# privefl/bigsnpr

Measured on AMD Instinct MI355X. Metric: SNP-cols/sec for bed_randomSVD k=20 (m*passes/wall), higher is better.
Workload: dtype i8 (2-bit codes x 24-bit (early block steps) / 16-bit (late block steps) fixed-point image of the fp64 basis in int8 slices, exact int32 MFMA accumulation; fp64 panel algebra and Rayleigh-Ritz)

## Files before the change

bigsnpr_amd/csrc/bsn_internal.hpp:

```cpp
#pragma once
#include <hip/hip_runtime.h>
#include <stdint.h>

#include <atomic>
#include <cstdarg>
#include <cstdio>
#include <functional>
#include <cstdlib>
#include <memory>
#include <stdexcept>
#include <string>
#include <vector>

#include "bigsnpr_hip.h"

namespace bsn {
inline const char *abl_getenv(const char *name) {
#ifdef BSN_ABLATION
  return getenv(name);
#else
  (void)name;
  return nullptr;
#endif
}
// ... 85 lines not shown
  void *comm = nullptr;
  int rank = 0, world = 1, device = 0;
  hipStream_t stream = nullptr;
  std::atomic<int> aborted{0};
  bool timing = false;
  struct Timed { hipEvent_t a, b; int cls; };
  std::vector<Timed> timed;
  std::vector<hipEvent_t> ev_pool;
  ~bsn_comm() {
    for (auto &t : timed) { (void)hipEventDestroy(t.a); (void)hipEventDestroy(t.b); }
    for (auto e : ev_pool) (void)hipEventDestroy(e);
  }
};

constexpr int kProfKinds = 6;
struct bsn_op {
  bsn_bed *bed = nullptr;
  int64_t n = 0, m = 0;
  bool rows_identity = true;
  bool cols_contig = true;
  bool no_na = false;
  bool na_skip_c = false, na_skip_p = false;
  bool stats_pending = false;
  bsn::DevBuf<int32_t> d_counts;
  bsn::DevBuf<int32_t> d_na;
  long long *h_na_total = nullptr;
  bool na_poll = false;
  int64_t col0 = 0;
  int slices = 4;
  int64_t passes = 0;
  const double *late_center = nullptr, *late_scale = nullptr;
  const double *preq_X = nullptr;
  int64_t preq_ldx = 0;
  int preq_nvec = 0, preq_S = 0;
  bool profile = false;
  int prof_kind_override = -1;
  std::vector<hipEvent_t> ev_begin, ev_end;
  std::vector<int> ev_kind;
  std::vector<char> ev_more;
  const void *prof_kernel[kProfKinds] = {};
  const void *last_kernel = nullptr;
  ~bsn_op() {
    for (auto e : ev_begin) (void)hipEventDestroy(e);
    for (auto e : ev_end) (void)hipEventDestroy(e);
    if (h_na_total) (void)hipHostFree(h_na_total);
  }
  bsn::DevBuf<int32_t> d_rows;
  bsn::DevBuf<int32_t> d_cols;
  bsn::DevBuf<double> d_center, d_scale;
  bsn::DevBuf<double> d_xfull;
  bsn::DevBuf<int8_t> d_q;
  bsn::DevBuf<int32_t> d_acc;
  bsn::DevBuf<double> d_meta;
  bsn::DevBuf<double> d_yfull;
};

struct bsn_bed {
  int64_t n = 0, m = 0, n_byte = 0, pitch = 0;
  int bits = 2;
  double v_off = 0.0, v_step = 1.0;
  bool generic = false;
  double *d_lut = nullptr;
  uint8_t *d_img = nullptr;
  uint8_t *d_tiled = nullptr;
  bool tiled_tried = false;
  size_t tiled_cap = 0;
  const uint8_t *h_map = nullptr;
  void *map_base = nullptr;
  size_t map_len = 0;
  int64_t slab_cols = 0;
  int fd_file = -1;
  bsn_bed *slab_img = nullptr;
  void *slab_stage = nullptr;
  bool streamed() const { return d_img == nullptr && h_map != nullptr; }
  uint8_t *d_smaj = nullptr;
  int64_t pitch_smaj = 0, rows_smaj = 0;
  bool smaj_tried = false;
  size_t smaj_cap = 0;
  void *smaj_job = nullptr;
  int64_t cap_m = 0;
  bsn_bed *sub = nullptr;
  uint64_t sub_key = 0;
  std::vector<int64_t> sub_cols, sub_rows;
  bool last_solve_on_sub = false;
  int device = 0;
  bool stream_borrowed = false;
  hipStream_t stream = nullptr;
  hipStream_t stream_up = nullptr;
  hipEvent_t ev_up = nullptr;
  hipEvent_t ev0 = nullptr, ev1 = nullptr;
  std::vector<int32_t> na_cnt;
  struct CountsCache {
    std::vector<int64_t> rows;
    std::vector<int32_t> cnt;
    void clear() {
      rows.clear();
      cnt.clear();
    }
  } counts_cache;
  struct StatsCache {
    bsn::DevBuf<int32_t> d_cnt;
    std::vector<uint8_t> known;
    int64_t n_known = 0;
    bsn::DevBuf<int32_t> d_cols;
    uint64_t cols_key = 0;
    void clear() {
// ... 141 lines not shown
```

bigsnpr_amd/csrc/matvec.hip:

```cpp
#include <cmath>
#include <cstdlib>

#include "bsn_internal.hpp"
#include "prodt_sparse.hpp"
#include <type_traits>

namespace bsn {

typedef int v4i __attribute__((ext_vector_type(4)));
typedef int v8i __attribute__((ext_vector_type(8)));

static thread_local const void *g_last_kernel = nullptr;
#define BSN_KLAUNCH(kern, ...)                 \
  do {                                         \
    g_last_kernel = (const void *)(kern);      \
    hipLaunchKernelGGL(kern, __VA_ARGS__);     \
  } while (0)

__device__ __forceinline__ uint32_t lut4(uint32_t lut, uint32_t sel) {
  return __builtin_amdgcn_perm(lut, lut, sel);
}
__device__ __forceinline__ uint32_t perm8(uint32_t hi, uint32_t lo, uint32_t sel) {
  return __builtin_amdgcn_perm(hi, lo, sel);
}

constexpr uint32_t kLutG0 = 0x00020100u;
constexpr uint32_t kLutNA = 0x01000000u;
constexpr uint32_t kLutHom2 = 0x00010000u;
constexpr uint32_t kLutHet = 0x00000100u;
constexpr uint32_t kLutRaw = 0xFFFFFFFFu;

struct VecMeta {
  unsigned long long absmax_bits;
  long long sum_hi, sum_lo;
  long long sum2_hi, sum2_lo;
  unsigned long long nonfinite;
  double qscale;
  double pad;
};
static_assert(sizeof(VecMeta) == 64, "VecMeta layout");

__global__ void k_meta_clear(VecMeta *meta, int nvec) {
  int v = blockIdx.x * blockDim.x + threadIdx.x;
  if (v < nvec) {
    VecMeta z = {};
    meta[v] = z;
  }
}

__global__ void k_scatter_rows(const double *X, int64_t ldx, const int32_t *rows, int64_t n,
                               double *xfull, int64_t ldf) {
  int64_t i = (int64_t)blockIdx.x * blockDim.x + threadIdx.x;
  int v = blockIdx.y;
  if (i >= n) return;
  atomicAdd(&xfull[(int64_t)rows[i] + v * ldf], X[i + v * ldx]);
}

// ... 129 lines not shown
#ifdef BSN_ABLATION
      const bool sm = (raw3 >> 8) == 2;
      const long long sgA = A < 0 ? -1 : 1, sgB = B < 0 ? -1 : 1;
      long long mA = A < 0 ? -A : A, mB = B < 0 ? -B : B;
#endif
#pragma unroll
      for (int s = 0; s < S; s++) {
#ifdef BSN_ABLATION
        const int8_t da = sm ? (int8_t)(sgA * (mA & 0x7F)) : (int8_t)(A & 0xFF), db = sm ? (int8_t)(sgB * (mB & 0x7F)) : (int8_t)(B & 0xFF);
        mA >>= 7;
        mB >>= 7;
#else
        const int8_t da = (int8_t)(A & 0xFF), db = (int8_t)(B & 0xFF);
#endif
        A = (A - da) >> 8;
        B = (B - db) >> 8;
        if constexpr (PERM == 2) {
          const int r = prodt_sparse_row(e), ba = prodt_sparse_byte(e, 0), bb = prodt_sparse_byte(e, 1);
          pk[r][s][ba >> 2] |= (uint32_t)(uint8_t)da << (8 * (ba & 3));
          pk[r][s][bb >> 2] |= (uint32_t)(uint8_t)db << (8 * (bb & 3));
        } else {
          pk[0][s][pos >> 2] |= (uint32_t)(uint8_t)da << (8 * (pos & 3));
          pk[1][s][pos >> 2] |= (uint32_t)(uint8_t)db << (8 * (pos & 3));
        }
      }
    }
    for (int p = 0; p < nplanes; p++)
#pragma unroll
      for (int s = 0; s < S; s++) {
#ifdef BSN_ABLATION
        const int col = (raw3 >> 8) == 1 ? s * (int)gridDim.y + v : v * S + s;
#else
        const int col = v * S + s;
#endif
        int8_t *dst = q + ((kb * nplanes + p) * ncol + col) * 16;
        *(uint4 *)dst = p == 0 ? uint4{pk[0][s][0], pk[0][s][1], pk[0][s][2], pk[0][s][3]}
                               : uint4{pk[1][s][0], pk[1][s][1], pk[1][s][2], pk[1][s][3]};
      }
  }
  for (int off = 32; off > 0; off >>= 1) {
    shi += __shfl_down(shi, off); slo += __shfl_down(slo, off);
    shi2 += __shfl_down(shi2, off); slo2 += __shfl_down(slo2, off);
  }
  if (tid == 0) {
    atomicAdd((unsigned long long *)&meta[v].sum_hi, (unsigned long long)shi);
    atomicAdd((unsigned long long *)&meta[v].sum_lo, (unsigned long long)slo);
    if (mode >= 1) {
      atomicAdd((unsigned long long *)&meta[v].sum2_hi, (unsigned long long)shi2);
      atomicAdd((unsigned long long *)&meta[v].sum2_lo, (unsigned long long)slo2);
    }
  }
}

template <int NB, int NPLANE, int KC, bool RAW0, bool STATS, bool CONTIG, int ABL = 0, int TILES = 2,
          int WAVES = 8, int MINW = 1, int TAG = 0, bool TILED = false, int SGB = 0, bool NASKIP = false>
__global__ __launch_bounds__(64 * WAVES, MINW) void k_cprod(const uint8_t *__restrict__ img, int64_t pitch,
                                               const int32_t *__restrict__ cols, int64_t col0,
                                               int64_t m, const int8_t *__restrict__ xq,
                                               int32_t *__restrict__ acc_out, int64_t m_out,
                                               uint32_t lutA, uint32_t lutB, uint32_t lutC,
                                               int32_t *__restrict__ counts, int32_t n_pad_samples) {
  constexpr int NCOL = 16 * NB;
  constexpr int LD = KC / 256;
  constexpr int XS = KC / 16 * NCOL;
  __shared__ uint4 xs[2][XS];
  const int tid = threadIdx.x, wave = tid >> 6, lane = tid & 63;
  const int c = lane & 15, g = lane >> 4;
  constexpr int NT = 64 * WAVES;
  const int64_t wg_base = (int64_t)blockIdx.x * (WAVES * 16 * TILES);
  const int64_t snp_base = wg_base + wave * (16 * TILES);
  const uint8_t *rowp[TILES];
  uint32_t voff[TILES];
#pragma unroll
  for (int t = 0; t < TILES; t++) {
    int64_t j = snp_base + t * 16 + c;
    if (j > m - 1) j = m - 1;
    int64_t col = CONTIG ? col0 + j : (int64_t)cols[j];
    rowp[t] = img + col * pitch + g * 16;
    voff[t] = TILED ? (uint32_t)((((j - wg_base) >> 6) * (pitch >> 8)) * 16384 + (j & 63) * 256 + g * 16)
                    : (uint32_t)((j - wg_base) * pitch + g * 16);
  }
  static_assert(!TILED || (CONTIG && (WAVES * 16 * TILES) % 64 == 0), "streaming layout: whole 64-variant blocks");
  const __amdgpu_buffer_rsrc_t rs = __builtin_amdgcn_make_buffer_rsrc(
      (void *)(TILED ? img + (((col0 + wg_base) >> 6) * (pitch >> 8)) * 16384
                     : img + (col0 + (CONTIG ? wg_base : 0)) * pitch),
      0, 0x7fffffff, 0x00020000);
  typedef unsigned int v4u __attribute__((ext_vector_type(4)));
  auto gload = [&](const int t, const int off) -> uint4 {
    if constexpr (CONTIG) {
      constexpr int AUX = ((ABL & 64) ? 2 : 0) | ((ABL & 128) ? 16 : 0);
      const int soff = TILED ? ((off >> 8) << 14) + (off & 255) : off;
      const v4u r = __builtin_amdgcn_raw_buffer_load_b128(rs, (int)voff[t], soff, AUX);
      return uint4{r.x, r.y, r.z, r.w};
    } else {
      return *(const uint4 *)(rowp[t] + off);
    }
  };
  const int nchunks = (int)(pitch * 4 / KC);
  const uint4 *xq4 = (const uint4 *)xq;

  v4i acc[TILES][NPLANE][NB];
#pragma unroll
  for (int t = 0; t < TILES; t++)
#pragma unroll
    for (int p = 0; p < NPLANE; p++)
#pragma unroll
// ... 334 lines not shown
      T[3][r4] = perm8(hi23, hi01, 0x07060302u);
    }
    __builtin_amdgcn_sched_barrier(0);
    if (ABL & 32) {
#pragma unroll
      for (int r = 0; r < 16; r++) X[SET][r] += (uint32_t)jn2;
    } else {
      load(jn2, X[SET]);
    }
    __builtin_amdgcn_sched_barrier(0);
#pragma unroll
    for (int q = 0; q < 4; q++)
#pragma unroll
      for (int u0 = 0; u0 < 4; u0++) {
        v4i g0, na;
#pragma unroll
        for (int r4 = 0; r4 < 4; r4++) {
          const uint32_t sel = (T[q][r4] >> (2 * u0)) & 0x03030303u;
          if (ABL & 2) {
            g0[r4] = (int)T[q][r4];
            na[r4] = (int)(T[q][r4] ^ lutQ);
          } else {
            g0[r4] = RAWP ? (int)sel : (int)lut4(lutP, sel);
            if (HASQ) na[r4] = (int)lut4(lutQ, sel);
          }
        }
#pragma unroll
        for (int nb = 0; nb < NB; nb++) {
          if (ABL & 1) {
            asm volatile("" ::"v"(g0), "v"(na), "v"(aw[nb]), "v"(awc[nb]));
          } else {
            acc[q * 4 + u0][nb] = __builtin_amdgcn_mfma_i32_16x16x64_i8(aw[nb], g0, acc[q * 4 + u0][nb], 0, 0, 0);
            if (HASQ)
              acc[q * 4 + u0][nb] = __builtin_amdgcn_mfma_i32_16x16x64_i8(awc[nb], na, acc[q * 4 + u0][nb], 0, 0, 0);
          }
        }
      }
    ws[SET ^ 1][wtid] = wreg;
    __syncthreads();
  };
  for (int64_t jb = j0; jb < j1; jb += 128) {
    step(std::integral_constant<int, 0>{}, jb);
    if (jb + 64 < j1) step(std::integral_constant<int, 1>{}, jb + 64);
  }
#pragma unroll
  for (int u = 0; u < 16; u++) {
    const int64_t i = wbase + sg * 16 + u;
#pragma unroll
    for (int nb = 0; nb < NB; nb++)
      *(v4i *)(acc_out + (((int64_t)by * n_pad + i) * NCOL + nb * 16 + 4 * g)) = acc[u][nb];
  }
}

template <int NB, bool HASQ, int TILES = 2, int WAVES = 16, int TAG = 0, int SGB = 3, bool NASKIP = false, bool SPARSE = false>
__global__ __launch_bounds__(64 * WAVES) void k_prodT(const uint8_t *__restrict__ simg, int64_t rows_t, int64_t chunk0,
                                                      int nchunks, int cps,
                                                      const int8_t *__restrict__ wq, int32_t *__restrict__ acc_out,
                                                      int64_t n_pad, uint32_t lutQ, int seg_bs, int seg_stride, int seg_off) {
  constexpr int KC = 512, NCOL = 16 * NB, LD = KC / 256;
  constexpr int XS = KC / 16 * 2 * NCOL;
  constexpr int NT = 64 * WAVES, NX = XS / NT;
  static_assert(XS % NT == 0 && NX >= 1 && NX <= 4, "digit staging");
  __shared__ uint4 xs[2][XS];
  const int tid = threadIdx.x, wave = tid >> 6, lane = tid & 63;
  const int c = lane & 15, g = lane >> 4;
  const unsigned bx = seg_bs > 0 ? (blockIdx.x / (unsigned)seg_bs) * (unsigned)seg_stride + (unsigned)seg_off + blockIdx.x % (unsigned)seg_bs
                                 : blockIdx.x;
  const int64_t wg_base = (int64_t)bx * (WAVES * 16 * TILES);
  const int64_t row_base = wg_base + wave * (16 * TILES);
  uint32_t voff[TILES];
#pragma unroll
  for (int t = 0; t < TILES; t++) {
    int64_t i = row_base + t * 16 + c;
    if (i > rows_t - 1) i = rows_t - 1;
    voff[t] = (uint32_t)((i - wg_base) * (KC / 4) + g * 16);
  }
  const int ch_begin = (int)blockIdx.y * cps;
  int ch_end = ch_begin + cps;
  if (ch_end > nchunks) ch_end = nchunks;
  if (ch_begin >= ch_end) return;
  if (wg_base >= rows_t) return;
  const int64_t chunk_stride = rows_t * (KC / 4);
  const uint8_t *const base0 = simg + ((chunk0 + ch_begin) * rows_t + wg_base) * (KC / 4);
  typedef unsigned int v4u __attribute__((ext_vector_type(4)));
  auto gload = [&](const int t, const int ch, const int off) -> uint4 {
    const __amdgpu_buffer_rsrc_t rs =
        __builtin_amdgcn_make_buffer_rsrc((void *)(base0 + (int64_t)ch * chunk_stride), 0, 0x7fffffff, 0x00020000);
    const v4u r = __builtin_amdgcn_raw_buffer_load_b128(rs, (int)voff[t], off, 0);
    return uint4{r.x, r.y, r.z, r.w};
  };
  const int nch = ch_end - ch_begin;
  const uint4 *xq4 = (const uint4 *)wq + (int64_t)ch_begin * XS;

  v4i acc[TILES][NB];
#pragma unroll
  for (int t = 0; t < TILES; t++)
#pragma unroll
    for (int nb = 0; nb < NB; nb++) acc[t][nb] = v4i{0, 0, 0, 0};
  uint4 ga[2][TILES][LD];
  uint4 xr0 = {0, 0, 0, 0}, xr1 = {0, 0, 0, 0}, xr2 = {0, 0, 0, 0}, xr3 = {0, 0, 0, 0};
#pragma unroll
  for (int t = 0; t < TILES; t++)
#pragma unroll
    for (int it = 0; it < LD; it++) ga[0][t][it] = gload(t, 0, it * 64);
#pragma unroll
  for (int x = 0; x < NX; x++) xs[0][tid + x * NT] = xq4[tid + x * NT];
#pragma unroll
  for (int t = 0; t < TILES; t++)
#pragma unroll
    for (int it = 0; it < LD; it++) ga[1][t][it] = gload(t, nch > 1 ? 1 : 0, it * 64);
  __syncthreads();
// ... 83 lines not shown
          for (int p = 0; p < NP; p++)
#pragma unroll
            for (int nb = 0; nb < NB; nb++) bv[p][nb] = bn[p][nb];
        }
      }
    }
#pragma unroll
    for (int t = 0; t < TILES; t++)
#pragma unroll
      for (int it = 0; it < LD; it++) ga[SET][t][it] = gload(t, ch2, it * 64);
    if constexpr (SGB & 1) {
      constexpr int VSTEP = TILES * (SPARSE ? 18 : 7 + (HASQ ? 4 : 0)), MSTEP = TILES * (SPARSE ? NB : NP * NB);
      __builtin_amdgcn_sched_group_barrier(0x100, NP * NB, 0);
      __builtin_amdgcn_sched_group_barrier(0x002, SPARSE ? 9 : 7, 0);
      auto slots = [&](auto self, auto IC) {
        constexpr int i = decltype(IC)::value;
        if constexpr (i < MSTEP) {
          constexpr int nv = VSTEP * (i + 1) / MSTEP - VSTEP * i / MSTEP;
          __builtin_amdgcn_sched_group_barrier(0x008, 1, 0);
          if constexpr (nv > 0) __builtin_amdgcn_sched_group_barrier(0x002, nv, 0);
          self(self, std::integral_constant<int, i + 1>{});
        }
      };
#pragma unroll
      for (int stp = 0; stp < LD * 4; stp++) {
        __builtin_amdgcn_sched_group_barrier(0x100, NP * NB, 0);
        slots(slots, std::integral_constant<int, 0>{});
      }
      __builtin_amdgcn_sched_group_barrier(0x020, TILES * LD, 0);
    }
    __builtin_amdgcn_sched_barrier(0);
    if constexpr (SGB & 2) __builtin_amdgcn_s_setprio(0);
    xs[SET ^ 1][tid] = xr0;
    if constexpr (NX > 1) xs[SET ^ 1][tid + NT] = xr1;
    if constexpr (NX > 2) xs[SET ^ 1][tid + 2 * NT] = xr2;
    if constexpr (NX > 3) xs[SET ^ 1][tid + 3 * NT] = xr3;
    __syncthreads();
  };
  for (int ch = 0; ch < nch; ch += 2) {
    chunk(std::integral_constant<int, 0>{}, ch);
    if (ch + 1 < nch) chunk(std::integral_constant<int, 1>{}, ch + 1);
  }
#pragma unroll
  for (int t = 0; t < TILES; t++)
#pragma unroll
    for (int r = 0; r < 4; r++) {
      const int64_t i = row_base + t * 16 + g * 4 + r;
      if (i < n_pad) {
#pragma unroll
        for (int nb = 0; nb < NB; nb++)
          acc_out[((int64_t)blockIdx.y * n_pad + i) * NCOL + nb * 16 + c] = acc[t][nb][r];
      }
    }
}

template <int NCOL>
__global__ __launch_bounds__(256) void k_prod_final(const int32_t *__restrict__ acc, int64_t n_pad, int ky, int S, int nv,
                             const VecMeta *meta, const int32_t *rows, int64_t n, double *Y,
                             int64_t ldy, int sub_const, double beta, int64_t blk_rows = 0) {
  int64_t i = (int64_t)blockIdx.x * blockDim.x + threadIdx.x;
  if (i >= n) return;
  int64_t i2 = rows ? (int64_t)rows[i] : i;
  if (i2 < 0) {
    for (int v = 0; v < nv; v++) Y[(i / blk_rows * nv + v) * blk_rows + i % blk_rows] = 0.0;
    return;
  }
  long long d[NCOL];
#pragma unroll
  for (int c = 0; c < NCOL; c++) d[c] = 0;
  for (int k = 0; k < ky; k++) {
    const int4 *a = (const int4 *)(acc + ((int64_t)k * n_pad + i2) * NCOL);
#pragma unroll
    for (int c4 = 0; c4 < NCOL / 4; c4++) {
      int4 t = a[c4];
      d[4 * c4 + 0] += t.x;
      d[4 * c4 + 1] += t.y;
      d[4 * c4 + 2] += t.z;
      d[4 * c4 + 3] += t.w;
    }
  }
  for (int v = 0; v < nv; v++) {
    double r = 0;
    for (int s = S - 1; s >= 0; s--) {
      long long dv = 0;
#pragma unroll
      for (int c = 0; c < NCOL; c++) dv = (c == v * S + s) ? d[c] : dv;
      r = r * 256.0 + (double)dv;
    }
    double C = sub_const ? (double)meta[v].sum2_hi * 16777216.0 + (double)meta[v].sum2_lo : 0.0;
    double qs = meta[v].qscale;
    double y = qs > 0 ? (r - C) / qs : 0.0;
    if (meta[v].nonfinite) y = __longlong_as_double(0x7ff8000000000000LL);
    if (blk_rows > 0)
      Y[(i / blk_rows * nv + v) * blk_rows + i % blk_rows] = y;
    else
      Y[i + v * ldy] = beta != 0.0 ? beta * Y[i + v * ldy] + y : y;
  }
}

__device__ __forceinline__ uint32_t val8m(uint32_t w, uint32_t &na) {
  const uint32_t t = w ^ 0x80808080u;
  const uint32_t y = (t & 0x7F7F7F7Fu) + 0x7F7F7F7Fu;
  const uint32_t z = ~(y | t | 0x7F7F7F7Fu);
  na = z >> 7;
  return w & ~(z | (z - na));
}
// ... 181 lines not shown
    }
  }
}

void require_bits(const bsn_bed *b, int bits, const char *what) {
  if (b->bits != bits)
    fail("%s is not available for this handle: it needs %s", what,
         bits == 2 ? "a 2-bit genotype image (.bed, or an FBM.code256 whose codes decode to 0 / 1 / 2 / NA)"
                   : "a byte (dosage) image");
}

void prof_begin(bsn_op *op, int kind, bool more) {
  if (!op->profile) return;
  if (op->prof_kind_override >= 0) kind = op->prof_kind_override;
  op->ev_more.push_back(more);
  hipEvent_t a, b;
  BSN_HIP(hipEventCreate(&a));
  BSN_HIP(hipEventCreate(&b));
  op->ev_begin.push_back(a);
  op->ev_end.push_back(b);
  op->ev_kind.push_back(kind);
  BSN_HIP(hipEventRecord(a, op->bed->stream));
}
void prof_end(bsn_op *op) {
  if (!op->profile) return;
  BSN_HIP(hipEventRecord(op->ev_end.back(), op->bed->stream));
  op->prof_kernel[op->ev_kind.back() % kProfKinds] = g_last_kernel;
}
void prof_collect(bsn_op *op, double ms[kProfKinds], int count[kProfKinds]) {
  for (int k = 0; k < kProfKinds; k++) ms[k] = 0, count[k] = 0;
  for (size_t i = 0; i < op->ev_begin.size(); i++) {
    float t = 0;
    if (hipEventSynchronize(op->ev_end[i]) == hipSuccess &&
        hipEventElapsedTime(&t, op->ev_begin[i], op->ev_end[i]) == hipSuccess) {
      ms[op->ev_kind[i]] += t;
      if (!op->ev_more[i]) count[op->ev_kind[i]]++;
    }
    (void)hipEventDestroy(op->ev_begin[i]);
    (void)hipEventDestroy(op->ev_end[i]);
  }
  (void)hipGetLastError();
  op->ev_begin.clear();
  op->ev_end.clear();
  op->ev_kind.clear();
  op->ev_more.clear();
}

constexpr int kMaxCols = 48;
static int pick_nb(int ncols_needed) { return ncols_needed <= 16 ? 1 : ncols_needed <= 32 ? 2 : 3; }
static bool nb3_allowed() {
  static const bool on = getenv("BSN_NO_NB3") == nullptr;
  return on;
}
constexpr int kMetaVecs = 32;
static VecMeta *meta_buffer(bsn_op *op) {
  return (VecMeta *)op->d_meta.ensure((size_t)kMetaVecs * 8 + (size_t)kMetaVecs * 256 * 2);
}
static inline int64_t n_padded(const bsn_bed *b) { return b->bits == 8 ? b->pitch : b->pitch * 4; }

static void quantise(bsn_op *op, const double *d_X, int64_t ldx, int64_t len, int64_t len_pad,
                     int nvec, int mode, int S, int ncol, int permute, int exact_int,
                     VecMeta *meta, int8_t *q, const double *d_W2 = nullptr) {
  hipStream_t st = op->bed->stream;
  const bool bytes = op->bed->bits == 8;
  const double vstep = bytes ? op->bed->v_step : 1.0, voff = bytes ? op->bed->v_off : 0.0;
  int raw3 = (!bytes && mode == 1) ? 1 : 0;
#ifdef BSN_ABLATION
  if (const char *dg = getenv("BSN_DIGITS")) raw3 |= atoi(dg) << 8;
#endif
  if (bytes) permute = 0;
  if (permute == 2 && !(mode == 1 && (raw3 & 1))) fail("internal: the interleaved digit rows are the scaled product's");
  double *part = (double *)(meta + kMetaVecs);
  int gx = 0;
  if (exact_int) {
    hipLaunchKernelGGL(k_meta_clear, dim3(1), dim3(64), 0, st, meta, nvec);
  } else {
    gx = (int)((len + 1023) / 1024);
    if (gx > 256) gx = 256;
    hipLaunchKernelGGL(k_absmax, dim3(gx, nvec), dim3(1024), 0, st, d_X, ldx, len,
                       mode == 1 ? op->d_center.p : mode == 2 ? d_W2 : nullptr,
                       mode == 1 ? op->d_scale.p : nullptr, mode, meta, part, vstep, voff, raw3);
  }
  int64_t nblk = len_pad / 16;
  const double *qc = mode == 1 ? op->d_center.p : mode == 2 ? d_W2 : nullptr;
  const double *qsc = mode == 1 ? op->d_scale.p : nullptr;
  const dim3 qgrid((unsigned)((nblk + 63) / 64), nvec);
#define BSN_QUANT(SV)                                                                                  \
  case SV:                                                                                             \
    if (permute == 2)                                                                                  \
      hipLaunchKernelGGL((k_quant<SV, 2>), qgrid, dim3(64), 0, st, d_X, ldx, len, len_pad, qc, qsc, mode, \
                         ncol, meta, q, vstep, voff, raw3, part, gx);                                  \
    else if (permute)                                                                                  \
      hipLaunchKernelGGL((k_quant<SV, 1>), qgrid, dim3(64), 0, st, d_X, ldx, len, len_pad, qc, qsc, mode, \
                         ncol, meta, q, vstep, voff, raw3, part, gx);                                  \
    else                                                                                               \
      hipLaunchKernelGGL((k_quant<SV, 0>), qgrid, dim3(64), 0, st, d_X, ldx, len, len_pad, qc, qsc, mode, \
                         ncol, meta, q, vstep, voff, raw3, part, gx);                                  \
    break;
  switch (S) {
    BSN_QUANT(1) BSN_QUANT(2) BSN_QUANT(3) BSN_QUANT(4) BSN_QUANT(5) BSN_QUANT(6) BSN_QUANT(7) BSN_QUANT(8)
    default: fail("slices must be in 1..8");
  }
#undef BSN_QUANT
  BSN_HIP(hipGetLastError());
}

static const double *scatter_rows_if_needed(bsn_op *op, const double *d_X, int64_t *ldx,
                                            int nvec) {
  if (op->rows_identity) return d_X;
  bsn_bed *b = op->bed;
  double *xf = op->d_xfull.ensure((size_t)b->n * nvec);
  BSN_HIP(hipMemsetAsync(xf, 0, (size_t)b->n * nvec * sizeof(double), b->stream));
  hipLaunchKernelGGL(k_scatter_rows, dim3((unsigned)((op->n + 255) / 256), nvec), dim3(256), 0,
                     b->stream, d_X, *ldx, op->d_rows.p, op->n, xf, b->n);
  BSN_HIP(hipGetLastError());
  *ldx = b->n;
  return xf;
}

#ifdef BSN_ABLATION
static int tune_variant() {
  static int v = -1;
  if (v < 0) {
    const char *e = getenv("BSN_TUNE");
    v = e ? atoi(e) : 0;
  }
  return v;
}
#endif

#pragma clang fp contract(off)
__global__ void k_binom_scale(const int32_t *counts, int64_t m, double *center, double *scale) {
  int64_t j = (int64_t)blockIdx.x * blockDim.x + threadIdx.x;
  if (j >= m) return;
  const int4 c = *(const int4 *)(counts + 4 * j);
  const double sumX = (double)(c.y + 2 * c.z);
  const double nona = (double)(c.x + c.y + c.z);
  const double af = sumX / (2.0 * nona);
  center[j] = 2.0 * af;
  scale[j] = sqrt(2.0 * af * (1.0 - af));
}
#pragma clang fp contract(on)

__global__ __launch_bounds__(256) void k_stats_summary(const int32_t *counts, int64_t m, int64_t n, int32_t *na,
                                                       unsigned long long *out) {
  long long s = 0, bad = 0;
  for (int64_t j = (int64_t)blockIdx.x * 256 + threadIdx.x; j < m; j += (int64_t)gridDim.x * 256) {
    const int4 c = *(const int4 *)(counts + 4 * j);
    s += c.w;
    na[j] = c.w;
    if (2 * ((int64_t)c.x + c.y + c.z) < n) bad++;
  }
  for (int off = 32; off > 0; off >>= 1) {
    s += __shfl_down(s, off);
    bad += __shfl_down(bad, off);
  }
// ... 421 lines not shown
      if (c < 6 && c < nchunks && nchunks >= 6) continue;
      const int64_t W = wgx * c;
      const double fill = (double)W / ((double)ncu * (double)((W + ncu - 1) / ncu));
      const double score = fill - slab_cost * c;
      if (score > best_score + 1e-9) best_score = score, best = c;
    }
    ky = best;
#ifdef BSN_ABLATION
    if (const char *e = getenv("BSN_KY_T")) ky = std::max(1, std::min(atoi(e), (int)nchunks));
#endif
    const int64_t ky_min2 = (m_pad + 2499999) / 2500000;
    if (ky < ky_min2) ky = (int)ky_min2;
    smaj_cps = (int)((nchunks + ky - 1) / ky);
    ky = (int)((nchunks + smaj_cps - 1) / smaj_cps);
  }
  if (!smaj) {
    if (ky > steps) ky = (int)steps;
    if (ky > 64) ky = 64;
  }
  if (ky < 1) ky = 1;
  if (smaj && (int64_t)ky * smaj_cps < m_pad / 512) fail("internal: the slabs of k_prodT do not cover the variants");
  if (b->bits == 2 && pick_nb((nvec < vmax ? nvec : vmax) * S) == 1) {
    const int ncol_max = 16 * pick_nb((nvec < vmax ? nvec : vmax) * S);
    int64_t cap = (int64_t)(0.04 * (double)m_pad / (32.0 * ncol_max));
    if (cap < 1) cap = 1;
    if (ky > cap) ky = (int)cap;
    int best = ky;
    double best_fill = 0.0;
    for (int c = ky; c >= 1 && 2 * c >= ky; c--) {
      const int64_t W = wgx * c;
      const double fill = (double)W / (512.0 * (double)((W + 511) / 512));
      if (fill > best_fill + 1e-9) best_fill = fill, best = c;
    }
    ky = best;
  }
#ifdef BSN_ABLATION
  if (!smaj) {
    if (const char *e = getenv("BSN_KY")) ky = atoi(e);
    if (ky > steps) ky = (int)steps;
    if (ky < 1) ky = 1;
  }
#endif
  const int64_t ky_min = (m_pad + 2499999) / 2500000;
  if (ky < ky_min && !smaj) ky = (int)ky_min;
  int64_t mc = round_up((steps + ky - 1) / ky, 1) * 64;
  if (!smaj) ky = (int)((m_pad + mc - 1) / mc);
  const bool has_q = lutQ != 0u && !(op->no_na && lutQ == kLutNA);
  const bool sparse_ok = smaj && has_q && getenv("BSN_NO_SPARSE_PROD") == nullptr &&
                         ldexp(3.0 * (double)m_pad, 8 * S - 1) < 9007199254740992.0;
  for (int v0 = 0; v0 < nvec; v0 += vmax) {
    int nv = nvec - v0 < vmax ? nvec - v0 : vmax;
    int NB = pick_nb(nv * S), ncol = 16 * NB;
    const bool sparse = sparse_ok && NB == 3 && !op->na_skip_p;
    int8_t *q = op->d_q.ensure((size_t)(npad > m_pad ? npad : m_pad) * kMaxCols * 2);
    size_t acc_need = (size_t)ky * npad * ncol;
    if (acc_need < (size_t)2 * op->m * kMaxCols) acc_need = (size_t)2 * op->m * kMaxCols;
    int32_t *acc = op->d_acc.ensure(acc_need);
    quantise(op, d_X + (int64_t)v0 * ldx, ldx, op->m, m_pad, nv, mode, S, ncol, smaj && NB >= 2 ? (sparse ? 2 : 1) : 0, 0, meta, q,
             d_W2 ? d_W2 + (int64_t)v0 * ldx : nullptr);
    dim3 grid((unsigned)wgx, (unsigned)ky);
    prof_begin(op, NB == 3 ? 5 : 1);
    if (smaj && NB >= 2) {
      const int nchunks = (int)(m_pad / 512);
      const bool warm = op->prof_kind_override == 3;
#define BSN_PRODT_(NBV, HASQV, TAGV, GRID, BS, STRIDE, OFF)                                                          \
  BSN_KLAUNCH((k_prodT<NBV, HASQV, 2, 16, TAGV>), GRID, dim3(1024), 0, b->stream, b->d_smaj, b->rows_smaj, op->col0 / 512, \
              nchunks, smaj_cps, q, acc, npad, lutQ, BS, STRIDE, OFF)
#ifdef BSN_ABLATION
      static const int nb3p = getenv("BSN_NB3") ? atoi(getenv("BSN_NB3")) : 0;
#define BSN_PRODT3(HASQV, GRID, BS, STRIDE, OFF)                                                                      \
  do {                                                                                                               \
    if (nb3p & 4)                                                                                                    \
      BSN_KLAUNCH((k_prodT<3, HASQV, 2, 16, 0, 0>), GRID, dim3(1024), 0, b->stream, b->d_smaj, b->rows_smaj, op->col0 / 512, \
                  nchunks, smaj_cps, q, acc, npad, lutQ, BS, STRIDE, OFF);                                           \
    else BSN_PRODT_(3, HASQV, 0, GRID, BS, STRIDE, OFF);                                                             \
  } while (0)
#else
#define BSN_PRODT3(HASQV, GRID, BS, STRIDE, OFF) BSN_PRODT_(3, HASQV, 0, GRID, BS, STRIDE, OFF)
#endif
#define BSN_PRODT_SKIP(NBV, GRID, BS, STRIDE, OFF)                                                                   \
  BSN_KLAUNCH((k_prodT<NBV, true, 2, 16, 0, 0, true>), GRID, dim3(1024), 0, b->stream, b->d_smaj, b->rows_smaj,       \
              op->col0 / 512, nchunks, smaj_cps, q, acc, npad, lutQ, BS, STRIDE, OFF)
#define BSN_PRODT_SPARSE(TAGV, GRID, BS, STRIDE, OFF)                                                                \
  BSN_KLAUNCH((k_prodT<3, true, 2, 16, TAGV, 3, false, true>), GRID, dim3(1024), 0, b->stream, b->d_smaj,  \
              b->rows_smaj, op->col0 / 512, nchunks, smaj_cps, q, acc, npad, lutQ, BS, STRIDE, OFF)
#define BSN_PRODT(HASQV, TAGV, GRID, BS, STRIDE, OFF)                                                                \
  do {                                                                                                               \
    if (HASQV && sparse) {                                                                \
      BSN_PRODT_SPARSE(TAGV, GRID, BS, STRIDE, OFF);                                                                 \
    } else if (HASQV && op->na_skip_p) {         \
      if (NB == 2) BSN_PRODT_SKIP(2, GRID, BS, STRIDE, OFF);                                                         \
      else BSN_PRODT_SKIP(3, GRID, BS, STRIDE, OFF);                                                                 \
    } else if (NB == 2) BSN_PRODT_(2, HASQV, TAGV, GRID, BS, STRIDE, OFF);                                           \
    else BSN_PRODT3(HASQV, GRID, BS, STRIDE, OFF);                                                                   \
  } while (0)
      if (sg) {
        for (int sidx = 0; sidx < sg->nseg; sidx++) {
          const ProdSegment &sgm = sg->segs[sidx];
          const dim3 gs((unsigned)(sg->pieces * sgm.bs), (unsigned)ky);
          if (sidx > 0) prof_begin(op, NB == 3 ? 5 : 1, true);
          if (has_q) BSN_PRODT(true, 0, gs, sgm.bs, sg->stride, sgm.off);
          else BSN_PRODT(false, 0, gs, sgm.bs, sg->stride, sgm.off);
          BSN_HIP(hipGetLastError());
          prof_end(op);
          const int64_t rows_s = (int64_t)sgm.bs * 512, tot = rows_s * sg->pieces;
          if (NB == 2)
            hipLaunchKernelGGL((k_prod_final<32>), dim3((unsigned)((tot + 255) / 256)), dim3(256), 0, b->stream, acc, npad, ky,
                               S, nv, meta, sgm.d_rows, tot, sgm.d_out, (int64_t)0, sub_const, 0.0, rows_s);
          else
            hipLaunchKernelGGL((k_prod_final<48>), dim3((unsigned)((tot + 255) / 256)), dim3(256), 0, b->stream, acc, npad, ky,
                               S, nv, meta, sgm.d_rows, tot, sgm.d_out, (int64_t)0, sub_const, 0.0, rows_s);
          BSN_HIP(hipGetLastError());
          (*sg->after)(sidx);
        }
        op->passes++;
        sg->done = true;
        continue;
      }
      if (has_q) { if (warm) BSN_PRODT(true, 1, grid, 0, 0, 0); else BSN_PRODT(true, 0, grid, 0, 0, 0); }
      else { if (warm) BSN_PRODT(false, 1, grid, 0, 0, 0); else BSN_PRODT(false, 0, grid, 0, 0, 0); }
#undef BSN_PRODT
#undef BSN_PRODT_SPARSE
#undef BSN_PRODT_SKIP
#undef BSN_PRODT3
#undef BSN_PRODT_
      BSN_HIP(hipGetLastError());
    } else if (NB > 2) {
      fail("internal: three column blocks without the sample-major copy");
    } else if (b->bits == 8) {
      if (mode != 1) fail("internal: plane products are not defined on a byte image");
      const dim3 grid8 = grid;
      const int64_t npad8 = npad;
      const int32_t *cols8 = op->d_cols.p;
#define BSN_PROD8(NBV, NAV, CV)                                                                          \
  BSN_KLAUNCH((k_prod8<NBV, NAV, CV>), grid8, dim3(256), 0, b->stream, b->d_img, b->pitch, cols8, \
                     op->col0, m_pad, mc, q, acc, npad8)
      if (NB == 1) {
        if (op->no_na) { if (op->cols_contig) BSN_PROD8(1, false, true); else BSN_PROD8(1, false, false); }
        else { if (op->cols_contig) BSN_PROD8(1, true, true); else BSN_PROD8(1, true, false); }
      } else {
        if (op->no_na) { if (op->cols_contig) BSN_PROD8(2, false, true); else BSN_PROD8(2, false, false); }
        else { if (op->cols_contig) BSN_PROD8(2, true, true); else BSN_PROD8(2, true, false); }
      }
#undef BSN_PROD8
      BSN_HIP(hipGetLastError());
    } else
    if (op->cols_contig) {
      if (NB == 1) launch_prod<1, true>(op, grid, m_pad, mc, q, acc, npad, lutP, lutQ, has_q);
      else launch_prod<2, true>(op, grid, m_pad, mc, q, acc, npad, lutP, lutQ, has_q);
    } else {
      if (NB == 1) launch_prod<1, false>(op, grid, m_pad, mc, q, acc, npad, lutP, lutQ, has_q);
      else launch_prod<2, false>(op, grid, m_pad, mc, q, acc, npad, lutP, lutQ, has_q);
    }
    prof_end(op);
    op->last_kernel = g_last_kernel;
    op->passes++;
    if (NB == 1)
      hipLaunchKernelGGL((k_prod_final<16>), dim3((unsigned)((op->n + 255) / 256)), dim3(256), 0, b->stream,
                         acc, npad, ky, S, nv, meta, op->rows_identity ? nullptr : op->d_rows.p, op->n,
                         d_Y + (int64_t)v0 * ldy, ldy, sub_const, beta);
    else if (NB == 2)
      hipLaunchKernelGGL((k_prod_final<32>), dim3((unsigned)((op->n + 255) / 256)), dim3(256), 0, b->stream,
                         acc, npad, ky, S, nv, meta, op->rows_identity ? nullptr : op->d_rows.p, op->n,
                         d_Y + (int64_t)v0 * ldy, ldy, sub_const, beta);
    else
      hipLaunchKernelGGL((k_prod_final<48>), dim3((unsigned)((op->n + 255) / 256)), dim3(256), 0, b->stream,
                         acc, npad, ky, S, nv, meta, op->rows_identity ? nullptr : op->d_rows.p, op->n,
                         d_Y + (int64_t)v0 * ldy, ldy, sub_const, beta);
    BSN_HIP(hipGetLastError());
  }
}

__global__ void k_cprod_raw_final(const int32_t *acc, int64_t m, int ncol, int S, const VecMeta *meta,
                                  double *P, double *Q, int64_t ld) {
  int64_t j = (int64_t)blockIdx.x * blockDim.x + threadIdx.x;
  int v = blockIdx.y;
  if (j >= m) return;
  const double qs = meta[v].qscale;
  const double inv = qs > 0 ? 1.0 / qs : 0.0;
  double p = horner_sub(acc + j * ncol + v * S, acc + (m + j) * ncol + v * S, 3, S) * inv,
         q = horner(acc + (m + j) * ncol + v * S, S) * inv;
  if (meta[v].nonfinite) p = q = __longlong_as_double(0x7ff8000000000000LL);
  P[j + v * ld] = p;
  Q[j + v * ld] = q;
}

void op_cprod_raw(bsn_op *op, const double *d_X, int64_t ldx, int nvec, double *d_P, double *d_Q,
                  int64_t ld) {
  require_bits(op->bed, 2, "the plane sums of multLinReg");
  op->preq_X = nullptr;
  bsn_bed *b = op->bed;
  const int S = op->slices;
  const int vmax = 32 / S;
  if (nvec <= 0) return;
  const double *xsrc = scatter_rows_if_needed(op, d_X, &ldx, nvec);
  const int64_t npad = n_padded(b);
  VecMeta *meta = meta_buffer(op);
  for (int v0 = 0; v0 < nvec; v0 += vmax) {
    int nv = nvec - v0 < vmax ? nvec - v0 : vmax;
    int NB = pick_nb(nv * S), ncol = 16 * NB;
    int8_t *q = op->d_q.ensure((size_t)npad * kMaxCols * 2);
    int32_t *acc = op->d_acc.ensure((size_t)2 * op->m * kMaxCols);
    quantise(op, xsrc + (int64_t)v0 * ldx, ldx, b->n, npad, nv, 0, S, ncol, 1, 0, meta, q);
    launch_cprod<2, true, false>(op, NB, q, acc, kLutRaw, kLutNA, 0);
    op->passes++;
    hipLaunchKernelGGL(k_cprod_raw_final, dim3((unsigned)((op->m + 255) / 256), nv), dim3(256), 0,
                       b->stream, acc, op->m, ncol, S, meta, d_P + (int64_t)v0 * ld,
                       d_Q + (int64_t)v0 * ld, ld);
    BSN_HIP(hipGetLastError());
  }
// ... 127 lines not shown
```

Before: 37.94 million.

## Fold k_prod_final into k_prodT via last-arriver epilogue; row-batched quantizer

Adds a last-block-arrives epilogue to k_prodT. The final workgroup along the y (split-K) dimension for each row block sums the partial int32 accumulators, rebuilds the fp64 result from the slices and writes Y directly, so the separate k_prod_final launch is skipped when the sample-major path is used with identity rows. It also adds k_quant_rows, which handles four vectors per 256-thread block, preloads the next vector's values and reuses the loaded center and scale, replacing the per-vector 64-thread quantize grid. The cost is an atomic arrival counter, extra threadfences, and serial epilogue work inside one block per row tile.

```diff
diff --git a/bigsnpr_amd/csrc/bsn_internal.hpp b/bigsnpr_amd/csrc/bsn_internal.hpp
--- a/bigsnpr_amd/csrc/bsn_internal.hpp
+++ b/bigsnpr_amd/csrc/bsn_internal.hpp
@@ -161,6 +161,7 @@
   bsn::DevBuf<int8_t> d_q;
   bsn::DevBuf<int32_t> d_acc;
   bsn::DevBuf<double> d_meta;
+  bsn::DevBuf<unsigned> d_arrive;
   bsn::DevBuf<double> d_yfull;
 };
 
diff --git a/bigsnpr_amd/csrc/matvec.hip b/bigsnpr_amd/csrc/matvec.hip
--- a/bigsnpr_amd/csrc/matvec.hip
+++ b/bigsnpr_amd/csrc/matvec.hip
@@ -3,6 +3,7 @@
 
 #include "bsn_internal.hpp"
 #include "prodt_sparse.hpp"
+#include "prod_fin.hpp"
 #include <type_traits>
 
 namespace bsn {
@@ -238,6 +239,146 @@
   }
 }
 
+template <int S, int PERM>
+__global__ __launch_bounds__(256) void k_quant_rows(const double *__restrict__ X, int64_t ldx, int64_t len,
+                                                    int64_t len_pad, const double *__restrict__ center,
+                                                    const double *__restrict__ scale, int mode, int ncol, int nvec,
+                                                    VecMeta *meta, int8_t *__restrict__ q, double vstep, double voff,
+                                                    int raw3, const double *__restrict__ part, int gx) {
+  __shared__ double sa_all[4][64 * 17], sb_all[4][64 * 17];
+  const int tid = threadIdx.x & 63, wave = threadIdx.x >> 6;
+  double *const sa = sa_all[wave], *const sb = sb_all[wave];
+  const int64_t kb = (int64_t)blockIdx.x * 64 + tid;
+  const int nplanes = mode >= 1 ? 2 : 1;
+  double xa[16], xc[16], xs[16];
+#pragma unroll
+  for (int it = 0; it < 16; it++) {
+    const int64_t k = (int64_t)blockIdx.x * 1024 + it * 64 + tid;
+    const bool in = k < len;
+    xc[it] = 0.0;
+    xs[it] = 1.0;
+    if (mode == 1) {
+      if (in && scale) xs[it] = scale[k];
+      if (in && center) xc[it] = center[k];
+    }
+    xa[it] = in && wave < nvec ? X[k + wave * ldx] : 0.0;
+  }
+  for (int v0 = 0; v0 < nvec; v0 += 4) {
+    const int v = v0 + wave;
+    const bool on = v < nvec;
+    double qs = 1.0;
+    if (on && gx > 0) {
+      double mx = 0, bad = 0;
+      for (int t = tid; t < gx; t += 64) {
+        mx = fmax(mx, part[((int64_t)v * gx + t) * 2]);
+        bad += part[((int64_t)v * gx + t) * 2 + 1];
+      }
+      for (int off = 32; off > 0; off >>= 1) {
+        mx = fmax(mx, __shfl_xor(mx, off));
+        bad += __shfl_xor(bad, off);
+      }
+      qs = 0.0;
+      if (mx > 0) {
+        int e;
+        frexp(ldexp(0.99, 8 * S - 1) / mx, &e);
+        qs = ldexp(1.0, e - 1);
+      }
+      if (blockIdx.x == 0 && tid == 0) {
+        meta[v].absmax_bits = (unsigned long long)__double_as_longlong(mx);
+        meta[v].nonfinite = (unsigned long long)bad;
+      }
+    }
+    if (on && blockIdx.x == 0 && tid == 0) meta[v].qscale = qs;
+    if (on) {
+      if (mode == 2) {
+#pragma unroll
+        for (int it = 0; it < 16; it++) {
+          const int64_t k = (int64_t)blockIdx.x * 1024 + it * 64 + tid;
+          xc[it] = k < len && center ? center[k + v * ldx] : 0.0;
+        }
+      }
+#pragma unroll
+      for (int it = 0; it < 16; it++) {
+        const int t = it * 64 + tid;
+        double a = xa[it], b = 0;
+        if (mode == 1) {
+          a = a / xs[it];
+          b = (xc[it] - voff) * a;
+          a *= vstep;
+        } else if (mode == 2) {
+          b = xc[it];
+        }
+        if (!(fabs(a) <= 1.79e308)) a = 0;
+        if (!(fabs(b) <= 1.79e308)) b = 0;
+        sa[t + (t >> 4)] = a * qs;
+        sb[t + (t >> 4)] = b * qs;
+      }
+      if (v + 4 < nvec) {
+#pragma unroll
+        for (int it = 0; it < 16; it++) {
+          const int64_t k = (int64_t)blockIdx.x * 1024 + it * 64 + tid;
+          xa[it] = k < len ? X[k + (v + 4) * ldx] : 0.0;
+        }
+      }
+    }
+    __syncthreads();
+    long long shi = 0, slo = 0, shi2 = 0, slo2 = 0;
+    if (on && kb * 16 < len_pad) {
+      uint32_t pk[2][S][4];
+#pragma unroll
+      for (int p = 0; p < 2; p++)
+#pragma unroll
+        for (int s = 0; s < S; s++)
+#pragma unroll
+          for (int w = 0; w < 4; w++) pk[p][s][w] = 0;
+#pragma unroll
+      for (int e = 0; e < 16; e++) {
+        long long A = llrint(sa[tid * 17 + e]), B = llrint(sb[tid * 17 + e]);
+        shi += A >> 24; slo += A & 0xFFFFFF;
+        shi2 += B >> 24; slo2 += B & 0xFFFFFF;
+        if ((raw3 & 1) && PERM != 2) B -= 3 * A;
+        const int pos = PERM == 1 ? ((e & 3) * 4 + (e >> 2)) : e;
+#pragma unroll
+        for (int s = 0; s < S; s++) {
+          const int8_t da = (int8_t)(A & 0xFF), db = (int8_t)(B & 0xFF);
+          A = (A - da) >> 8;
+          B = (B - db) >> 8;
+          if constexpr (PERM == 2) {
+            const int r = prodt_sparse_row(e), ba = prodt_sparse_byte(e, 0), bb = prodt_sparse_byte(e, 1);
+            pk[r][s][ba >> 2] |= (uint32_t)(uint8_t)da << (8 * (ba & 3));
+            pk[r][s][bb >> 2] |= (uint32_t)(uint8_t)db << (8 * (bb & 3));
+          } else {
+            pk[0][s][pos >> 2] |= (uint32_t)(uint8_t)da << (8 * (pos & 3));
+            pk[1][s][pos >> 2] |= (uint32_t)(uint8_t)db << (8 * (pos & 3));
+          }
+        }
+      }
+      for (int p = 0; p < nplanes; p++)
+#pragma unroll
+        for (int s = 0; s < S; s++) {
+          int8_t *dst = q + ((kb * nplanes + p) * ncol + v * S + s) * 16;
+          *(uint4 *)dst = p == 0 ? uint4{pk[0][s][0], pk[0][s][1], pk[0][s][2], pk[0][s][3]}
+                                 : uint4{pk[1][s][0], pk[1][s][1], pk[1][s][2], pk[1][s][3]};
+        }
+    }
+    if (on) {
+      for (int off = 32; off > 0; off >>= 1) {
+        shi += __shfl_down(shi, off); slo += __shfl_down(slo, off);
+        shi2 += __shfl_down(shi2, off); slo2 += __shfl_down(slo2, off);
+      }
+      if (tid == 0) {
+        atomicAdd((unsigned long long *)&meta[v].sum_hi, (unsigned long long)shi);
+        atomicAdd((unsigned long long *)&meta[v].sum_lo, (unsigned long long)slo);
+        if (mode >= 1) {
+          atomicAdd((unsigned long long *)&meta[v].sum2_hi, (unsigned long long)shi2);
+          atomicAdd((unsigned long long *)&meta[v].sum2_lo, (unsigned long long)slo2);
+        }
+      }
+    }
+    __syncthreads();
+  }
+}
+
 template <int NB, int NPLANE, int KC, bool RAW0, bool STATS, bool CONTIG, int ABL = 0, int TILES = 2,
           int WAVES = 8, int MINW = 1, int TAG = 0, bool TILED = false, int SGB = 0, bool NASKIP = false>
 __global__ __launch_bounds__(64 * WAVES, MINW) void k_cprod(const uint8_t *__restrict__ img, int64_t pitch,
@@ -678,11 +819,21 @@
   }
 }
 
-template <int NB, bool HASQ, int TILES = 2, int WAVES = 16, int TAG = 0, int SGB = 3, bool NASKIP = false, bool SPARSE = false>
+struct ProdFin {
+  unsigned *arrive;
+  const VecMeta *meta;
+  double *Y;
+  int64_t ldy, n;
+  int S, nv, sub_const;
+  double beta;
+};
+template <int NB, bool HASQ, int TILES = 2, int WAVES = 16, int TAG = 0, int SGB = 3, bool NASKIP = false, bool SPARSE = false,
+          bool FIN = false>
 __global__ __launch_bounds__(64 * WAVES) void k_prodT(const uint8_t *__restrict__ simg, int64_t rows_t, int64_t chunk0,
                                                       int nchunks, int cps,
                                                       const int8_t *__restrict__ wq, int32_t *__restrict__ acc_out,
-                                                      int64_t n_pad, uint32_t lutQ, int seg_bs, int seg_stride, int seg_off) {
+                                                      int64_t n_pad, uint32_t lutQ, int seg_bs, int seg_stride, int seg_off,
+                                                      ProdFin fin) {
   constexpr int KC = 512, NCOL = 16 * NB, LD = KC / 256;
   constexpr int XS = KC / 16 * 2 * NCOL;
   constexpr int NT = 64 * WAVES, NX = XS / NT;
@@ -872,6 +1023,65 @@
           acc_out[((int64_t)blockIdx.y * n_pad + i) * NCOL + nb * 16 + c] = acc[t][nb][r];
       }
     }
+  if constexpr (FIN) {
+    static_assert(TILES * WAVES * 16 == 512 && NT == 1024, "the epilogue's halves of 256 rows");
+    __shared__ int last;
+    __threadfence();
+    __syncthreads();
+    if (tid == 0) {
+      const unsigned before = atomicAdd(&fin.arrive[bx], 1u);
+      last = before + 1u == gridDim.y;
+      if (last) fin.arrive[bx] = 0u;
+    }
+    __syncthreads();
+    if (!last) return;
+    __threadfence();
+    static_assert(kProdFinRows * NCOL * 8 == sizeof(xs) && kProdFinRows * (NCOL / 4) == NB * NT, "the sums of a half");
+    long long *const ls = (long long *)&xs[0][0];
+    const int32_t *const part = acc_out;
+    for (int h = 0; h < 2; h++) {
+      const int64_t r0 = wg_base + h * kProdFinRows;
+#pragma unroll
+      for (int x = 0; x < NB; x++) {
+        const int it = tid + x * NT, r = prod_fin_item_row(it, NCOL), c4 = prod_fin_item_c4(it, NCOL);
+        const int64_t i = r0 + r;
+        if (i < fin.n) {
+          long long d0 = 0, d1 = 0, d2 = 0, d3 = 0;
+          const int4 *a = (const int4 *)(part + i * NCOL) + c4;
+          const int64_t slab = n_pad * (NCOL / 4);
+#pragma unroll 4
+          for (int k = 0; k < (int)gridDim.y; k++) {
+            const int4 t = a[k * slab];
+            d0 += t.x;
+            d1 += t.y;
+            d2 += t.z;
+            d3 += t.w;
+          }
+          ls[prod_fin_slot(r, 4 * c4 + 0, NCOL)] = d0;
+          ls[prod_fin_slot(r, 4 * c4 + 1, NCOL)] = d1;
+          ls[prod_fin_slot(r, 4 * c4 + 2, NCOL)] = d2;
+          ls[prod_fin_slot(r, 4 * c4 + 3, NCOL)] = d3;
+        }
+      }
+      __syncthreads();
+      for (int it = tid; it < fin.nv * kProdFinRows; it += NT) {
+        const int v = it / kProdFinRows, r = it % kProdFinRows;
+        const int64_t i = r0 + r;
+        if (i >= fin.n) continue;
+        double rr = 0;
+        for (int s = fin.S - 1; s >= 0; s--) {
+          const long long dv = ls[prod_fin_slot(r, v * fin.S + s, NCOL)];
+          rr = rr * 256.0 + (double)dv;
+        }
+        double C = fin.sub_const ? (double)fin.meta[v].sum2_hi * 16777216.0 + (double)fin.meta[v].sum2_lo : 0.0;
+        double qs = fin.meta[v].qscale;
+        double y = qs > 0 ? (rr - C) / qs : 0.0;
+        if (fin.meta[v].nonfinite) y = __longlong_as_double(0x7ff8000000000000LL);
+        fin.Y[i + v * fin.ldy] = fin.beta != 0.0 ? fin.beta * fin.Y[i + v * fin.ldy] + y : y;
+      }
+      __syncthreads();
+    }
+  }
 }
 
 template <int NCOL>
@@ -1159,6 +1369,7 @@
   static const bool on = getenv("BSN_NO_NB3") == nullptr;
   return on;
 }
+static bool fused_panel_off() { return getenv("BSN_NO_FUSED_PANEL") != nullptr; }
 constexpr int kMetaVecs = 32;
 static VecMeta *meta_buffer(bsn_op *op) {
   return (VecMeta *)op->d_meta.ensure((size_t)kMetaVecs * 8 + (size_t)kMetaVecs * 256 * 2);
@@ -1192,8 +1403,18 @@
   const double *qc = mode == 1 ? op->d_center.p : mode == 2 ? d_W2 : nullptr;
   const double *qsc = mode == 1 ? op->d_scale.p : nullptr;
   const dim3 qgrid((unsigned)((nblk + 63) / 64), nvec);
+  const bool rows_wg = !fused_panel_off() && (raw3 >> 8) == 0;
+  const dim3 rgrid((unsigned)((nblk + 63) / 64));
+#define BSN_QUANT_ROWS(SV, PV)                                                                         \
+  hipLaunchKernelGGL((k_quant_rows<SV, PV>), rgrid, dim3(256), 0, st, d_X, ldx, len, len_pad, qc, qsc, mode, ncol, nvec, \
+                     meta, q, vstep, voff, raw3, part, gx)
 #define BSN_QUANT(SV)                                                                                  \
   case SV:                                                                                             \
+    if (rows_wg) {                                                                                     \
+      if (permute == 2) BSN_QUANT_ROWS(SV, 2);                                                         \
+      else if (permute) BSN_QUANT_ROWS(SV, 1);                                                         \
+      else BSN_QUANT_ROWS(SV, 0);                                                                      \
+    } else                                                                                             \
     if (permute == 2)                                                                                  \
       hipLaunchKernelGGL((k_quant<SV, 2>), qgrid, dim3(64), 0, st, d_X, ldx, len, len_pad, qc, qsc, mode, \
                          ncol, meta, q, vstep, voff, raw3, part, gx);                                  \
@@ -1209,6 +1430,7 @@
     default: fail("slices must be in 1..8");
   }
 #undef BSN_QUANT
+#undef BSN_QUANT_ROWS
   BSN_HIP(hipGetLastError());
 }
 
@@ -1736,6 +1958,10 @@
     int nv = nvec - v0 < vmax ? nvec - v0 : vmax;
     int NB = pick_nb(nv * S), ncol = 16 * NB;
     const bool sparse = sparse_ok && NB == 3 && !op->na_skip_p;
+    bool fold = smaj && NB >= 2 && !sg && op->rows_identity && !fused_panel_off();
+#ifdef BSN_ABLATION
+    if (getenv("BSN_NB3")) fold = false;
+#endif
     int8_t *q = op->d_q.ensure((size_t)(npad > m_pad ? npad : m_pad) * kMaxCols * 2);
     size_t acc_need = (size_t)ky * npad * ncol;
     if (acc_need < (size_t)2 * op->m * kMaxCols) acc_need = (size_t)2 * op->m * kMaxCols;
@@ -1747,44 +1973,57 @@
     if (smaj && NB >= 2) {
       const int nchunks = (int)(m_pad / 512);
       const bool warm = op->prof_kind_override == 3;
-#define BSN_PRODT_(NBV, HASQV, TAGV, GRID, BS, STRIDE, OFF)                                                          \
-  BSN_KLAUNCH((k_prodT<NBV, HASQV, 2, 16, TAGV>), GRID, dim3(1024), 0, b->stream, b->d_smaj, b->rows_smaj, op->col0 / 512, \
-              nchunks, smaj_cps, q, acc, npad, lutQ, BS, STRIDE, OFF)
+      ProdFin fin{};
+      if (fold) {
+        if ((size_t)wgx > op->d_arrive.n) {
+          unsigned *ar = op->d_arrive.ensure((size_t)wgx);
+          BSN_HIP(hipMemsetAsync(ar, 0, (size_t)wgx * sizeof(unsigned), b->stream));
+        }
+        fin = ProdFin{op->d_arrive.p, meta, d_Y + (int64_t)v0 * ldy, ldy, op->n, S, nv, sub_const, beta};
+      }
+#define BSN_PRODT_(NBV, HASQV, TAGV, FINV, GRID, BS, STRIDE, OFF)                                                    \
+  BSN_KLAUNCH((k_prodT<NBV, HASQV, 2, 16, TAGV, 3, false, false, FINV>), GRID, dim3(1024), 0, b->stream, b->d_smaj,   \
+              b->rows_smaj, op->col0 / 512, nchunks, smaj_cps, q, acc, npad, lutQ, BS, STRIDE, OFF, fin)
 #ifdef BSN_ABLATION
       static const int nb3p = getenv("BSN_NB3") ? atoi(getenv("BSN_NB3")) : 0;
-#define BSN_PRODT3(HASQV, GRID, BS, STRIDE, OFF)                                                                      \
+#define BSN_PRODT3(HASQV, FINV, GRID, BS, STRIDE, OFF)                                                                \
   do {                                                                                                               \
     if (nb3p & 4)                                                                                                    \
-      BSN_KLAUNCH((k_prodT<3, HASQV, 2, 16, 0, 0>), GRID, dim3(1024), 0, b->stream, b->d_smaj, b->rows_smaj, op->col0 / 512, \
-                  nchunks, smaj_cps, q, acc, npad, lutQ, BS, STRIDE, OFF);                                           \
-    else BSN_PRODT_(3, HASQV, 0, GRID, BS, STRIDE, OFF);                                                             \
+      BSN_KLAUNCH((k_prodT<3, HASQV, 2, 16, 0, 0, false, false, FINV>), GRID, dim3(1024), 0, b->stream, b->d_smaj,    \
+                  b->rows_smaj, op->col0 / 512, nchunks, smaj_cps, q, acc, npad, lutQ, BS, STRIDE, OFF, fin);        \
+    else BSN_PRODT_(3, HASQV, 0, FINV, GRID, BS, STRIDE, OFF);                                                       \
   } while (0)
 #else
-#define BSN_PRODT3(HASQV, GRID, BS, STRIDE, OFF) BSN_PRODT_(3, HASQV, 0, GRID, BS, STRIDE, OFF)
+#define BSN_PRODT3(HASQV, FINV, GRID, BS, STRIDE, OFF) BSN_PRODT_(3, HASQV, 0, FINV, GRID, BS, STRIDE, OFF)
 #endif
-#define BSN_PRODT_SKIP(NBV, GRID, BS, STRIDE, OFF)                                                                   \
-  BSN_KLAUNCH((k_prodT<NBV, true, 2, 16, 0, 0, true>), GRID, dim3(1024), 0, b->stream, b->d_smaj, b->rows_smaj,       \
-              op->col0 / 512, nchunks, smaj_cps, q, acc, npad, lutQ, BS, STRIDE, OFF)
-#define BSN_PRODT_SPARSE(TAGV, GRID, BS, STRIDE, OFF)                                                                \
-  BSN_KLAUNCH((k_prodT<3, true, 2, 16, TAGV, 3, false, true>), GRID, dim3(1024), 0, b->stream, b->d_smaj,  \
-              b->rows_smaj, op->col0 / 512, nchunks, smaj_cps, q, acc, npad, lutQ, BS, STRIDE, OFF)
-#define BSN_PRODT(HASQV, TAGV, GRID, BS, STRIDE, OFF)                                                                \
+#define BSN_PRODT_SKIP(NBV, FINV, GRID, BS, STRIDE, OFF)                                                             \
+  BSN_KLAUNCH((k_prodT<NBV, true, 2, 16, 0, 0, true, false, FINV>), GRID, dim3(1024), 0, b->stream, b->d_smaj,        \
+              b->rows_smaj, op->col0 / 512, nchunks, smaj_cps, q, acc, npad, lutQ, BS, STRIDE, OFF, fin)
+#define BSN_PRODT_SPARSE(TAGV, FINV, GRID, BS, STRIDE, OFF)                                                          \
+  BSN_KLAUNCH((k_prodT<3, true, 2, 16, TAGV, 3, false, true, FINV>), GRID, dim3(1024), 0, b->stream, b->d_smaj,       \
+              b->rows_smaj, op->col0 / 512, nchunks, smaj_cps, q, acc, npad, lutQ, BS, STRIDE, OFF, fin)
+#define BSN_PRODT(HASQV, TAGV, FINV, GRID, BS, STRIDE, OFF)                                                          \
   do {                                                                                                               \
     if (HASQV && sparse) {                                                                \
-      BSN_PRODT_SPARSE(TAGV, GRID, BS, STRIDE, OFF);                                                                 \
+      BSN_PRODT_SPARSE(TAGV, FINV, GRID, BS, STRIDE, OFF);                                                           \
     } else if (HASQV && op->na_skip_p) {         \
-      if (NB == 2) BSN_PRODT_SKIP(2, GRID, BS, STRIDE, OFF);                                                         \
-      else BSN_PRODT_SKIP(3, GRID, BS, STRIDE, OFF);                                                                 \
-    } else if (NB == 2) BSN_PRODT_(2, HASQV, TAGV, GRID, BS, STRIDE, OFF);                                           \
-    else BSN_PRODT3(HASQV, GRID, BS, STRIDE, OFF);                                                                   \
+      if (NB == 2) BSN_PRODT_SKIP(2, FINV, GRID, BS, STRIDE, OFF);                                                   \
+      else BSN_PRODT_SKIP(3, FINV, GRID, BS, STRIDE, OFF);                                                           \
+    } else if (NB == 2) BSN_PRODT_(2, HASQV, TAGV, FINV, GRID, BS, STRIDE, OFF);                                     \
+    else BSN_PRODT3(HASQV, FINV, GRID, BS, STRIDE, OFF);                                                             \
+  } while (0)
+#define BSN_PRODT_F(HASQV, TAGV, GRID)                                                                               \
+  do {                                                                                                               \
+    if (fold) BSN_PRODT(HASQV, TAGV, true, GRID, 0, 0, 0);                                                           \
+    else BSN_PRODT(HASQV, TAGV, false, GRID, 0, 0, 0);                                                               \
   } while (0)
       if (sg) {
         for (int sidx = 0; sidx < sg->nseg; sidx++) {
           const ProdSegment &sgm = sg->segs[sidx];
           const dim3 gs((unsigned)(sg->pieces * sgm.bs), (unsigned)ky);
           if (sidx > 0) prof_begin(op, NB == 3 ? 5 : 1, true);
-          if (has_q) BSN_PRODT(true, 0, gs, sgm.bs, sg->stride, sgm.off);
-          else BSN_PRODT(false, 0, gs, sgm.bs, sg->stride, sgm.off);
+          if (has_q) BSN_PRODT(true, 0, false, gs, sgm.bs, sg->stride, sgm.off);
+          else BSN_PRODT(false, 0, false, gs, sgm.bs, sg->stride, sgm.off);
           BSN_HIP(hipGetLastError());
           prof_end(op);
           const int64_t rows_s = (int64_t)sgm.bs * 512, tot = rows_s * sg->pieces;
@@ -1801,8 +2040,9 @@
         sg->done = true;
         continue;
       }
-      if (has_q) { if (warm) BSN_PRODT(true, 1, grid, 0, 0, 0); else BSN_PRODT(true, 0, grid, 0, 0, 0); }
-      else { if (warm) BSN_PRODT(false, 1, grid, 0, 0, 0); else BSN_PRODT(false, 0, grid, 0, 0, 0); }
+      if (has_q) { if (warm) BSN_PRODT_F(true, 1, grid); else BSN_PRODT_F(true, 0, grid); }
+      else { if (warm) BSN_PRODT_F(false, 1, grid); else BSN_PRODT_F(false, 0, grid); }
+#undef BSN_PRODT_F
 #undef BSN_PRODT
 #undef BSN_PRODT_SPARSE
 #undef BSN_PRODT_SKIP
@@ -1839,7 +2079,8 @@
     prof_end(op);
     op->last_kernel = g_last_kernel;
     op->passes++;
-    if (NB == 1)
+    if (fold) {
+    } else if (NB == 1)
       hipLaunchKernelGGL((k_prod_final<16>), dim3((unsigned)((op->n + 255) / 256)), dim3(256), 0, b->stream,
                          acc, npad, ky, S, nv, meta, op->rows_identity ? nullptr : op->d_rows.p, op->n,
                          d_Y + (int64_t)v0 * ldy, ldy, sub_const, beta);
diff --git a/bigsnpr_amd/csrc/prod_fin.hpp b/bigsnpr_amd/csrc/prod_fin.hpp
--- /dev/null
+++ b/bigsnpr_amd/csrc/prod_fin.hpp
@@ -0,0 +1,17 @@
+#pragma once
+
+#if defined(__HIPCC__)
+#define BSN_FIN_HD __host__ __device__ __forceinline__
+#else
+#define BSN_FIN_HD inline
+#endif
+
+namespace bsn {
+
+constexpr int kProdFinRows = 256;
+
+BSN_FIN_HD int prod_fin_item_row(const int it, const int ncol) { return it / (ncol / 4); }
+BSN_FIN_HD int prod_fin_item_c4(const int it, const int ncol) { return it % (ncol / 4); }
+BSN_FIN_HD int prod_fin_slot(const int r, const int c, const int ncol) { return r * ncol + (c + r) % ncol; }
+
+}
```

After: 33.90 million. -10.6%, worse.
